# szhan227/text2protein

Measured on AMD Instinct MI355X. Metric: 6D backbone samples/sec (128-res, 1000-step), higher is better.
Workload: dtype f16; 1 GPU; cfg2: test_config.yml L=128 N=1000 chains/GPU=32 C=5 text_tokens=512 condition=none; step = 1 PC step (2 score evals + SDE updates); sample = 1000 PC steps; finite=True

## Files before the change

### text2protein_amd/csrc/attention.hip

```cpp
#include "t2p_kernels.h"

namespace t2p {

typedef float f32x16 __attribute__((ext_vector_type(16)));
typedef __bf16 bf16x8_t __attribute__((ext_vector_type(8)));
typedef _Float16 f16x8_t __attribute__((ext_vector_type(8)));

template <typename TC> struct AMma;
template <> struct AMma<bf16_t> {
  __device__ static inline void run(const uint4& a, const uint4& b, f32x16& c) {
    c = __builtin_amdgcn_mfma_f32_32x32x16_bf16(__builtin_bit_cast(bf16x8_t, a), __builtin_bit_cast(bf16x8_t, b), c, 0, 0, 0);
  }
};
template <> struct AMma<f16_t> {
  __device__ static inline void run(const uint4& a, const uint4& b, f32x16& c) {
    c = __builtin_amdgcn_mfma_f32_32x32x16_f16(__builtin_bit_cast(f16x8_t, a), __builtin_bit_cast(f16x8_t, b), c, 0, 0, 0);
  }
};

template <typename TC> __device__ inline uint32_t pack2(float a, float b);
template <> __device__ inline uint32_t pack2<bf16_t>(float a, float b) {
  return (uint32_t)f32_to_bf16_bits(a) | ((uint32_t)f32_to_bf16_bits(b) << 16);
}
template <> __device__ inline uint32_t pack2<f16_t>(float a, float b) {
// ... 181 lines not shown
  }

  const int qrow = q0 + lr;
  if (qrow < a.nq) {
    const float inv = 1.f / l;
    TC* orow = (TC*)a.out + (long)b * a.so_b + (long)qrow * a.ldo + (long)head * D;
#pragma unroll
    for (int tt = 0; tt < NT; ++tt)
#pragma unroll
      for (int g = 0; g < 4; ++g) {
        const int dv = tt * 32 + 8 * g + 4 * lh;
        uint2 u;
        u.x = pack2<TC>(o[tt][4 * g + 0] * inv, o[tt][4 * g + 1] * inv);
        u.y = pack2<TC>(o[tt][4 * g + 2] * inv, o[tt][4 * g + 3] * inv);
        *(uint2*)(orow + dv) = u;
      }
  }
}

template <typename TC, int D, bool VROW>
static int launch_flash_t(const FlashArgs& a, int B, int heads, hipStream_t s) {
  constexpr int smem = 2 * (64 * (D * 2 + 16) + (VROW ? 64 * (D == 32 ? 64 : (D == 64 ? 192 : 320)) : D * (64 * 2 + 8)));
  auto kern = attn_flash_kernel<TC, D, VROW>;
  T2P_TRY(ensure_dynamic_lds((const void*)kern, smem));
  dim3 grid((a.nq + 127) / 128, heads, B);
  hipEvent_t e0 = nullptr, e1 = nullptr;
  if (prof_on()) {
    T2P_HIP_CHECK(hipEventCreate(&e0));
    T2P_HIP_CHECK(hipEventCreate(&e1));
    T2P_HIP_CHECK(hipEventRecord(e0, s));
  }
  hipLaunchKernelGGL(kern, grid, dim3(256), smem, s, a);
  if (e0) {
    T2P_HIP_CHECK(hipEventRecord(e1, s));
    prof_attention(e0, e1, 4.0 * (double)a.nq * a.nk * D * heads * B);
  }
  T2P_HIP_CHECK(hipGetLastError());
  return T2P_OK;
}


struct StripArgs {
  const void* q; long ldq; long sq_b;
  const void* k; long ldk; long sk_b;
  const void* vt; long ldvt; long svt_b;
  void* out; long ldo; long so_b;
  int n;
  float scale_log2e;
  int ep, out_f32, r_lowp;
  const float* bias;
  const void* res; long ldr;
  float alpha;
  float* col_stats;
};

template <typename TC, int D, int NKT, bool FM = false>
__global__ __launch_bounds__(512) void attn_strip_kernel(const StripArgs a) {
  constexpr int QRS = D * 2 + 16;
  constexpr int KW = NKT * 32;
  constexpr int PRS = KW * 8 * 2 + 16;
  constexpr int CT = D / 256;
  constexpr int REGION = (64 * QRS > 64 * PRS) ? 64 * QRS : 64 * PRS;
  extern __shared__ __attribute__((aligned(16))) unsigned char smem[];
  float* st_max = (float*)(smem + REGION);
  float* st_sum = st_max + 8 * 64;

  const int tid = threadIdx.x, lane = tid & 63, wave = __builtin_amdgcn_readfirstlane(tid >> 6);
  const int lr = lane & 31, lh = lane >> 5;
  const int lid = xcd_logical_id((int)(blockIdx.x + gridDim.x * blockIdx.y), (int)(gridDim.x * gridDim.y));
  const int strip = lid % (int)gridDim.x, b = lid / (int)gridDim.x;
  const int q0 = strip * 64, n = a.n;
  const TC* Q = (const TC*)a.q + (long)b * a.sq_b;
  const TC* K = (const TC*)a.k + (long)b * a.sk_b;
  const TC* VT = (const TC*)a.vt + (long)b * a.svt_b;

  for (int i = tid; i < 64 * (D / 8); i += 512) {
    const int row = i / (D / 8), ch = i - row * (D / 8);
    uint4 v = make_uint4(0, 0, 0, 0);
    if (q0 + row < n) v = *(const uint4*)(Q + (long)(q0 + row) * a.ldq + ch * 8);
    *(uint4*)(smem + row * QRS + ch * 16) = v;
  }
  __syncthreads();

  const int key_w = wave * KW;
  const bool w_active = key_w < n;
  f32x16 sacc[NKT][2];
#pragma unroll
  for (int kt = 0; kt < NKT; ++kt)
#pragma unroll
    for (int qt = 0; qt < 2; ++qt)
#pragma unroll
      for (int v = 0; v < 16; ++v) sacc[kt][qt][v] = 0.f;
  if (w_active) {
    const TC* krow[NKT];
#pragma unroll
    for (int kt = 0; kt < NKT; ++kt) {
      int key = key_w + kt * 32 + lr;
      key = key < n ? key : n - 1;
      krow[kt] = K + (long)key * a.ldk + 16 * lh;
    }
#if defined(STRIP_FM_TIMING)
#define KLD(kt, S, j) (*(const uint4*)(K + ((((long)(key_w / 32 + (kt)) * (D / 32) + (S)) * 2 + (j)) * 64 + lane) * 8))
#else
#define KLD(kt, S, j) (FM ? *(const uint4*)(K + ((((long)(key_w / 32 + (kt)) * (D / 32) + (S)) * 2 + (j)) * 64 + lane) * 8) \
                          : *(const uint4*)(krow[kt] + 32 * (S) + 8 * (j)))
#endif
    const unsigned char* qb0 = smem + lr * QRS + 32 * lh;
    uint4 ka0[NKT][2], ka1[NKT][2];
#pragma unroll
    for (int kt = 0; kt < NKT; ++kt) {
      ka0[kt][0] = KLD(kt, 0, 0);
      ka0[kt][1] = KLD(kt, 0, 1);
    }
    auto sstep = [&](const uint4 (&ka)[NKT][2], int S) {
      uint4 qf[2][2];
#pragma unroll
      for (int qt = 0; qt < 2; ++qt)
#pragma unroll
        for (int j = 0; j < 2; ++j) qf[qt][j] = *(const uint4*)(qb0 + qt * 32 * QRS + S * 64 + j * 16);
#pragma unroll
      for (int kt = 0; kt < NKT; ++kt)
#pragma unroll
        for (int j = 0; j < 2; ++j)
#pragma unroll
          for (int qt = 0; qt < 2; ++qt) AMma<TC>::run(ka[kt][j], qf[qt][j], sacc[kt][qt]);
    };
    for (int S = 0; S < D / 32; S += 2) {
#pragma unroll
      for (int kt = 0; kt < NKT; ++kt) {
        ka1[kt][0] = KLD(kt, S + 1, 0);
        ka1[kt][1] = KLD(kt, S + 1, 1);
      }
      sstep(ka0, S);
      if (S + 2 < D / 32) {
#pragma unroll
        for (int kt = 0; kt < NKT; ++kt) {
          ka0[kt][0] = KLD(kt, S + 2, 0);
          ka0[kt][1] = KLD(kt, S + 2, 1);
        }
      }
      sstep(ka1, S + 1);
    }
  }

  float mloc[2] = {-INFINITY, -INFINITY};
  if (w_active) {
#pragma unroll
    for (int kt = 0; kt < NKT; ++kt) {
      const int kbase = key_w + kt * 32;
      if (kbase + 32 > n) {
#pragma unroll
        for (int v = 0; v < 16; ++v)
          if (kbase + (v & 3) + 8 * (v >> 2) + 4 * lh >= n) { sacc[kt][0][v] = -INFINITY; sacc[kt][1][v] = -INFINITY; }
      }
#pragma unroll
      for (int qt = 0; qt < 2; ++qt)
#pragma unroll
        for (int v = 0; v < 16; ++v) mloc[qt] = fmaxf(mloc[qt], sacc[kt][qt][v]);
    }
  }
#pragma unroll
  for (int qt = 0; qt < 2; ++qt) {
    mloc[qt] = fmaxf(mloc[qt], __shfl_xor(mloc[qt], 32, 64));
    if (lh == 0) st_max[wave * 64 + qt * 32 + lr] = mloc[qt];
  }
  __syncthreads();
  float mq[2], lsum[2] = {0.f, 0.f};
#pragma unroll
  for (int qt = 0; qt < 2; ++qt) {
    float m = st_max[qt * 32 + lr];
#pragma unroll
    for (int w = 1; w < 8; ++w) m = fmaxf(m, st_max[w * 64 + qt * 32 + lr]);
    mq[qt] = m * a.scale_log2e;
  }
  if (w_active) {
#pragma unroll
    for (int kt = 0; kt < NKT; ++kt)
#pragma unroll
      for (int qt = 0; qt < 2; ++qt) {
        unsigned char* prow = smem + (qt * 32 + lr) * PRS + (key_w + kt * 32 + 4 * lh) * 2;
#pragma unroll
        for (int g = 0; g < 4; ++g) {
          float e[4];
#pragma unroll
          for (int i = 0; i < 4; ++i) {
            e[i] = __builtin_amdgcn_exp2f(fmaf(sacc[kt][qt][4 * g + i], a.scale_log2e, -mq[qt]));
            lsum[qt] += e[i];
          }
          *(uint2*)(prow + 16 * g) = make_uint2(pack2<TC>(e[0], e[1]), pack2<TC>(e[2], e[3]));
        }
      }
  }
#pragma unroll
  for (int qt = 0; qt < 2; ++qt) {
    lsum[qt] += __shfl_xor(lsum[qt], 32, 64);
    if (lh == 0) st_sum[wave * 64 + qt * 32 + lr] = lsum[qt];
  }
  __syncthreads();
  float inv[2];
#pragma unroll
  for (int qt = 0; qt < 2; ++qt) {
    float l = st_sum[qt * 32 + lr];
#pragma unroll
    for (int w = 1; w < 8; ++w) l += st_sum[w * 64 + qt * 32 + lr];
    inv[qt] = 1.f / l;
  }

  f32x16 oacc[CT][2];
#pragma unroll
  for (int t = 0; t < CT; ++t)
#pragma unroll
    for (int qt = 0; qt < 2; ++qt)
#pragma unroll
      for (int v = 0; v < 16; ++v) oacc[t][qt][v] = 0.f;
  const int ch_w = wave * (D / 8);
  const TC* vrow[CT];
#pragma unroll
  for (int t = 0; t < CT; ++t) vrow[t] = VT + (long)(ch_w + t * 32 + lr) * a.ldvt + 16 * lh;
  const int nss = (n + 31) >> 5;
  auto vload = [&](int t, int S, int j) -> uint4 {
    const int key = 32 * S + 16 * lh + 8 * j;
#ifdef STRIP_FM_TIMING
    return key < n ? *(const uint4*)(VT + ((((long)(ch_w / 32 + t) * ((n + 31) >> 5) + S) * 2 + j) * 64 + lane) * 8) : make_uint4(0, 0, 0, 0);
#else
    if constexpr (FM) return *(const uint4*)(VT + ((((long)(ch_w / 32 + t) * (n >> 5) + S) * 2 + j) * 64 + lane) * 8);
    return key < n ? *(const uint4*)(vrow[t] + 32 * S + 8 * j) : make_uint4(0, 0, 0, 0);
#endif
  };
  uint4 va0[CT][2], va1[CT][2];
#pragma unroll
  for (int t = 0; t < CT; ++t) { va0[t][0] = vload(t, 0, 0); va0[t][1] = vload(t, 0, 1); }
  const unsigned char* pb0 = smem + lr * PRS + 32 * lh;
  auto pstep = [&](const uint4 (&va)[CT][2], int S) {
    uint4 pf[2][2];
#pragma unroll
    for (int qt = 0; qt < 2; ++qt)
#pragma unroll
      for (int j = 0; j < 2; ++j) pf[qt][j] = *(const uint4*)(pb0 + qt * 32 * PRS + S * 64 + j * 16);
#pragma unroll
    for (int t = 0; t < CT; ++t)
#pragma unroll
      for (int j = 0; j < 2; ++j)
#pragma unroll
        for (int qt = 0; qt < 2; ++qt) AMma<TC>::run(va[t][j], pf[qt][j], oacc[t][qt]);
  };
  for (int S = 0; S < nss; S += 2) {
    if (S + 1 < nss) {
#pragma unroll
      for (int t = 0; t < CT; ++t) { va1[t][0] = vload(t, S + 1, 0); va1[t][1] = vload(t, S + 1, 1); }
    }
    pstep(va0, S);
    if (S + 1 < nss) {
      if (S + 2 < nss) {
#pragma unroll
        for (int t = 0; t < CT; ++t) { va0[t][0] = vload(t, S + 2, 0); va0[t][1] = vload(t, S + 2, 1); }
      }
      pstep(va1, S + 1);
    }
  }

  if (!a.ep) {
#pragma unroll
    for (int qt = 0; qt < 2; ++qt) {
      const int qrow = q0 + qt * 32 + lr;
      if (qrow < n) {
        TC* orow = (TC*)a.out + (long)b * a.so_b + (long)qrow * a.ldo + ch_w;
#pragma unroll
        for (int t = 0; t < CT; ++t)
#pragma unroll
          for (int g = 0; g < 4; ++g) {
            uint2 u;
            u.x = pack2<TC>(oacc[t][qt][4 * g + 0] * inv[qt], oacc[t][qt][4 * g + 1] * inv[qt]);
            u.y = pack2<TC>(oacc[t][qt][4 * g + 2] * inv[qt], oacc[t][qt][4 * g + 3] * inv[qt]);
            *(uint2*)(orow + t * 32 + 8 * g + 4 * lh) = u;
          }
      }
    }
    return;
  }
#pragma unroll
  for (int t = 0; t < CT; ++t)
#pragma unroll
    for (int g = 0; g < 4; ++g) {
      const int ch = ch_w + t * 32 + 8 * g + 4 * lh;
      const float4 bs = a.bias ? *(const float4*)(a.bias + ch) : make_float4(0.f, 0.f, 0.f, 0.f);
      float cs[4] = {0.f, 0.f, 0.f, 0.f}, cq[4] = {0.f, 0.f, 0.f, 0.f};
#pragma unroll
      for (int qt = 0; qt < 2; ++qt) {
        const int qrow = q0 + qt * 32 + lr;
        if (qrow < n) {
          const long ro = (long)b * n * a.ldr + (long)qrow * a.ldr + ch;
          float r0 = 0.f, r1 = 0.f, r2 = 0.f, r3 = 0.f;
          if (a.res) {
            if (a.r_lowp) {
              union { uint2 u; TC e[4]; } x;
              x.u = *(const uint2*)((const TC*)a.res + ro);
              r0 = to_f32(x.e[0]); r1 = to_f32(x.e[1]); r2 = to_f32(x.e[2]); r3 = to_f32(x.e[3]);
            } else {
              const float4 x = *(const float4*)((const float*)a.res + ro);
              r0 = x.x; r1 = x.y; r2 = x.z; r3 = x.w;
            }
          }
          const float v0 = (oacc[t][qt][4 * g + 0] * inv[qt] + bs.x + r0) * a.alpha, v1 = (oacc[t][qt][4 * g + 1] * inv[qt] + bs.y + r1) * a.alpha;
          const float v2 = (oacc[t][qt][4 * g + 2] * inv[qt] + bs.z + r2) * a.alpha, v3 = (oacc[t][qt][4 * g + 3] * inv[qt] + bs.w + r3) * a.alpha;
          cs[0] += v0; cs[1] += v1; cs[2] += v2; cs[3] += v3;
          cq[0] += v0 * v0; cq[1] += v1 * v1; cq[2] += v2 * v2; cq[3] += v3 * v3;
          const long oo = (long)b * a.so_b + (long)qrow * a.ldo + ch;
          if (a.out_f32) *(float4*)((float*)a.out + oo) = make_float4(v0, v1, v2, v3);
          else *(uint2*)((TC*)a.out + oo) = make_uint2(pack2<TC>(v0, v1), pack2<TC>(v2, v3));
        }
      }
      if (a.col_stats) {
#pragma unroll
        for (int i = 0; i < 4; ++i)
#pragma unroll
          for (int sh = 1; sh < 32; sh <<= 1) { cs[i] += __shfl_xor(cs[i], sh, 64); cq[i] += __shfl_xor(cq[i], sh, 64); }
        if (lr == 0) {
          float* dst = a.col_stats + ((long)(b * (n >> 6) + strip) * D + ch) * 2;
          *(float4*)dst = make_float4(cs[0], cq[0], cs[1], cq[1]);
          *(float4*)(dst + 4) = make_float4(cs[2], cq[2], cs[3], cq[3]);
        }
      }
    }
}

bool g_attn_strip = true;
bool attention_strip_eligible(int dtype, int heads, int nq, int nk, int d, long ldq, long ldk, long ldvt, long ldo) {
  if (!g_attn_strip || dtype == DT_F32 || heads != 1 || nq != nk) return false;
  if (d != 256 && d != 512 && d != 1024) return false;
  if (nk < 8 || nk > 1024 || nk % 8 != 0) return false;
  if (d == 1024 && nk > 512) return false;
  return ldq % 8 == 0 && ldk % 8 == 0 && ldvt % 8 == 0 && ldvt >= nk && ldo % 4 == 0;
}

template <typename TC, int D, int NKT, bool FM = false>
static int launch_strip_t(const StripArgs& a, int B, hipStream_t s) {
  constexpr int QB = 64 * (D * 2 + 16), PB = 64 * (NKT * 32 * 8 * 2 + 16);
  constexpr int smem = (QB > PB ? QB : PB) + 2 * 8 * 64 * 4;
  static_assert(smem <= 160 * 1024, "attn_strip: LDS budget");
  auto kern = attn_strip_kernel<TC, D, NKT, FM>;
  T2P_TRY(ensure_dynamic_lds((const void*)kern, smem));
  hipEvent_t e0 = nullptr, e1 = nullptr;
  if (prof_on()) {
    T2P_HIP_CHECK(hipEventCreate(&e0));
    T2P_HIP_CHECK(hipEventCreate(&e1));
    T2P_HIP_CHECK(hipEventRecord(e0, s));
  }
  hipLaunchKernelGGL(kern, dim3((a.n + 63) / 64, B), dim3(512), smem, s, a);
  if (e0) {
    T2P_HIP_CHECK(hipEventRecord(e1, s));
    prof_attention(e0, e1, 4.0 * (double)a.n * a.n * D * B);
  }
  T2P_HIP_CHECK(hipGetLastError());
  return T2P_OK;
}

bool attention_strip_frag_major_ok(int dtype, int n, int d) {
  if ((dtype != DT_F16 && dtype != DT_BF16) || n % 32 != 0) return false;
  return (d == 512 && n > 512 && n <= 1024) || (d == 256 && n <= 256);
}
int launch_attention_strip(int dtype, const void* q, long ldq, const void* k, long ldk, const void* vt, long ldvt, void* out, long ldo,
                           int B, int n, int d, float scale, hipStream_t s, const StripEpilogue* ep) {
  T2P_REQUIRE(attention_strip_eligible(dtype, 1, n, n, d, ldq, ldk, ldvt, ldo), "wide-head attention: unsupported shape");
  T2P_REQUIRE(q && k && vt && out && B > 0 && scale > 0.f, "wide-head attention arguments");
  T2P_REQUIRE(((uintptr_t)q % 16) == 0 && ((uintptr_t)k % 16) == 0 && ((uintptr_t)vt % 16) == 0 && ((uintptr_t)out % 8) == 0,
              "wide-head attention: operands must be 16-byte aligned");
  StripArgs a;
  a.q = q; a.ldq = ldq; a.sq_b = (long)n * ldq;
  a.k = k; a.ldk = ldk; a.sk_b = (long)n * ldk;
  a.vt = vt; a.ldvt = ldvt; a.svt_b = (long)d * ldvt;
  a.out = out; a.ldo = ldo; a.so_b = (long)n * ldo;
  a.n = n;
  a.scale_log2e = scale * 1.44269504088896340736f;
  a.ep = ep ? 1 : 0; a.out_f32 = 0; a.r_lowp = 0; a.bias = nullptr; a.res = nullptr; a.ldr = 0; a.alpha = 1.f; a.col_stats = nullptr;
  if (ep) {
    T2P_REQUIRE(!ep->col_stats || n % 64 == 0, "wide-head attention: column statistics need whole 64-query strips");
    T2P_REQUIRE(!ep->residual || (ep->ldr % 4 == 0 && ((uintptr_t)ep->residual % 16) == 0), "wide-head attention: residual alignment");
    T2P_REQUIRE(((uintptr_t)out % 16) == 0 && ldo % 4 == 0, "wide-head attention: output alignment");
    a.out_f32 = ep->out_f32; a.r_lowp = ep->r_lowp; a.bias = ep->bias; a.res = ep->residual; a.ldr = ep->ldr; a.alpha = ep->alpha;
    a.col_stats = ep->col_stats;
  }
  const int nkt = n <= 256 ? 1 : (n <= 512 ? 2 : 4);
  if (ep && ep->frag_major) {
    T2P_REQUIRE(attention_strip_frag_major_ok(dtype, n, d), "wide-head attention: fragment-major operands need d = 512 with 512 < n <= 1024 or d = 256 with n <= 256, n % 32 == 0");
    a.sk_b = (long)n * d; a.svt_b = (long)n * d;
    if (d == 256) {
      if (dtype == DT_BF16) return launch_strip_t<bf16_t, 256, 1, true>(a, B, s);
      return launch_strip_t<f16_t, 256, 1, true>(a, B, s);
    }
    if (dtype == DT_BF16) return launch_strip_t<bf16_t, 512, 4, true>(a, B, s);
    return launch_strip_t<f16_t, 512, 4, true>(a, B, s);
  }
#define T2P_STRIP(TC, DD)                                                        \
  do {                                                                           \
    if (nkt == 1) return launch_strip_t<TC, DD, 1>(a, B, s);                     \
    if (nkt == 2) return launch_strip_t<TC, DD, 2>(a, B, s);                     \
    if constexpr (DD != 1024) return launch_strip_t<TC, DD, 4>(a, B, s);         \
  } while (0)
  if (dtype == DT_BF16) {
    if (d == 256) T2P_STRIP(bf16_t, 256);
    if (d == 512) T2P_STRIP(bf16_t, 512);
    if (d == 1024) T2P_STRIP(bf16_t, 1024);
  } else {
    if (d == 256) T2P_STRIP(f16_t, 256);
    if (d == 512) T2P_STRIP(f16_t, 512);
    if (d == 1024) T2P_STRIP(f16_t, 1024);
  }
#undef T2P_STRIP
  set_last_error("wide-head attention: no instantiation");
  return T2P_ERR_INVALID;
}

bool attention_flash_eligible(int dtype, int d, long ldq, long ldk, long ldvt, long ldo) {
  if (dtype == DT_F32) return false;
  if (d != 32 && d != 64 && d != 128) return false;
  return ldq % 8 == 0 && ldk % 8 == 0 && ldvt % 8 == 0 && ldo % 4 == 0;
}

int launch_attention_flash(int dtype, const void* q, long ldq, const void* k, long ldk, const void* vt, long ldvt,
                           void* out, int B, int heads, int nq, int nk, int d, float scale, hipStream_t s, bool v_rowmajor) {
  T2P_REQUIRE(attention_flash_eligible(dtype, d, ldq, ldk, ldvt, (long)heads * d), "flash attention: unsupported shape");
  T2P_REQUIRE(q && k && vt && out && B > 0 && heads > 0 && nq > 0 && nk > 0, "flash attention arguments");
  T2P_REQUIRE(scale > 0.f, "flash attention: the running maximum is taken on unscaled scores (scale must be positive)");
  T2P_REQUIRE(((uintptr_t)q % 16) == 0 && ((uintptr_t)k % 16) == 0 && ((uintptr_t)vt % 16) == 0 && ((uintptr_t)out % 8) == 0,
              "flash attention: operands must be 16-byte aligned");
  FlashArgs a;
  a.q = q; a.ldq = ldq; a.sq_b = (long)nq * ldq;
  a.k = k; a.ldk = ldk; a.sk_b = (long)nk * ldk;
  a.vt = vt; a.ldvt = ldvt; a.svt_b = v_rowmajor ? (long)nk * ldvt : (long)heads * d * ldvt;
  a.out = out; a.ldo = (long)heads * d; a.so_b = (long)nq * heads * d;
  a.nq = nq; a.nk = nk;
  a.scale_log2e = scale * 1.44269504088896340736f;
#define T2P_FLASH(TC, DD) return v_rowmajor ? launch_flash_t<TC, DD, true>(a, B, heads, s) : launch_flash_t<TC, DD, false>(a, B, heads, s)
  if (dtype == DT_BF16) {
    if (d == 32) T2P_FLASH(bf16_t, 32);
    if (d == 64) T2P_FLASH(bf16_t, 64);
    T2P_FLASH(bf16_t, 128);
  } else {
    if (d == 32) T2P_FLASH(f16_t, 32);
    if (d == 64) T2P_FLASH(f16_t, 64);
    T2P_FLASH(f16_t, 128);
  }
#undef T2P_FLASH
}

}
```

### text2protein_amd/csrc/capi.cpp

```cpp
#include <new>

#include "ddim.h"
#include "engine.h"
#include "sampler.h"
#include "train.h"

using namespace t2p;

#define API_BEGIN try {
#define API_END                                        \
  }                                                    \
  catch (const std::bad_alloc&) {                      \
    set_last_error("out of host memory");              \
    return T2P_ERR_STATE;                              \
  }                                                    \
  catch (const std::exception& ex) {                   \
    set_last_error(std::string("exception: ") + ex.what()); \
    return T2P_ERR_STATE;                              \
  }

namespace t2p { extern bool g_pre_conv_mfma, g_gn_apply_cols; void layer_profile_begin(); int layer_profile_end(std::string* out);
void debug_tap_set(int index, float* dst, long capacity); void debug_tap_shape(long out[4]); }
extern "C" {

// ... 640 lines not shown
  T2P_REQUIRE(npairs < (1u << 30), "encode_6d: too many block pairs");
  struct Scratch {
    int32_t* p = nullptr; hipStream_t s;
    ~Scratch() { if (p) { (void)hipStreamSynchronize(s); (void)hipFree(p); } }
  } dev;
  dev.s = s;
  T2P_HIP_CHECK(hipMalloc(&dev.p, up.size() * 4));
  T2P_HIP_CHECK(hipMemcpyAsync(dev.p, up.data(), up.size() * 4, hipMemcpyHostToDevice, s));
  return launch_encode6d(xyz, nres, atom_ok, batch, channels, L, dev.p, dev.p + 4 * (size_t)n_blocks, (int)npairs, coords_6d, mask_pair, s);
  API_END
}

int t2p_op_embedding_gather(const void* table, int table_dtype, const int32_t* ids, float* out, int64_t n_tokens, int dim, int vocab,
                            int32_t* bad_flag, void* stream) {
  API_BEGIN
  return launch_embedding_gather(table, table_dtype, ids, out, n_tokens, dim, vocab, bad_flag, (hipStream_t)stream);
  API_END
}

int t2p_op_apply_mask(float* x, const uint8_t* mask, const float* x_initial, int64_t n, void* stream) {
  API_BEGIN
  return launch_apply_mask(x, mask, x_initial, n, (hipStream_t)stream);
  API_END
}

int t2p_debug_set(int key, int value) {
  if (key == 10) { g_op_ws_bytes = (size_t)value << 20; return T2P_OK; }
  if (key == 11) { set_gemm_force_nsplit(value); return T2P_OK; }
  if (key == 12) { set_gemm_midsplit(value != 0); return T2P_OK; }
  if (key == 13) { g_gn_small = value != 0; return T2P_OK; }
  if (key == 14) { g_lowp_residual = value != 0; return T2P_OK; }
  if (key == 15) { set_gemm_thin_conv(value != 0); return T2P_OK; }
  if (key == 17) { g_gn_apply16 = value != 0; return T2P_OK; }
  if (key == 20) { g_layernorm16 = value != 0; return T2P_OK; }
  if (key == 21) { set_gemm_up4(value != 0); return T2P_OK; }
  if (key == 22) { set_gemm_deep_ring(value != 0); return T2P_OK; }
  if (key == 23) { set_gemm_fuse_shortcut(value != 0); return T2P_OK; }
  if (key == 25) { g_qkv_fused = value != 0; return T2P_OK; }
  if (key == 26) { t2p::g_pre_conv_mfma = value != 0; return T2P_OK; }
  if (key == 27) { t2p::g_gn_apply_cols = value != 0; return T2P_OK; }
  if (key == 28) { set_gemm_post_gn(value != 0); return T2P_OK; }
  if (key == 29) { t2p::g_attn_strip = value != 0; return T2P_OK; }
  if (key == 36) { t2p::g_small_conv = value != 0; return T2P_OK; }
  if (key == 38) { t2p::g_pre_conv_split = value != 0; return T2P_OK; }
  if (key == 39) { t2p::g_st_fuse = value != 0; return T2P_OK; }
  if (key == 40) { t2p::g_st_tail = value != 0; return T2P_OK; }
  if (key == 41) { t2p::g_small_conv_fm = value != 0; return T2P_OK; }
  if (key == 42) { t2p::g_st_ffpo = value != 0; return T2P_OK; }
  if (key == 43) { t2p::g_st_tail_rows = value; return T2P_OK; }
  if (key == 45) { t2p::g_attn_fm = value != 0; return T2P_OK; }
  if (key == 46) { t2p::g_attn_proj = value != 0; return T2P_OK; }
  if (key == 47) { set_gemm_dxs(value != 0); return T2P_OK; }
  if (key == 48) { t2p::g_train_plumbing16 = value != 0; return T2P_OK; }
  if (key == 34) { set_gemm_a_norm(value != 0); return T2P_OK; }
  if (key == 32) { g_attn_merged = value != 0; return T2P_OK; }
  if (key == 33) { g_ffpo_merged = value != 0; return T2P_OK; }
  if (key == 30) { set_gemm_split_consts(value, 0); return T2P_OK; }
  if (key == 31) { set_gemm_split_consts(0, value); return T2P_OK; }
  if (key == 0) set_gemm_dma(value != 0);
  else if (key == 1) {
#ifndef T2P_ABLATION
    if (value & ~(128 | 256 | 4096 | 8192)) {
      set_last_error("ablation bits that skip work exist only in a -DT2P_ABLATION build");
      return T2P_ERR_INVALID;
    }
#endif
    set_gemm_debug(value);
  }
  else if (key == 2) set_gemm_geom(value);
  else if (key == 3) set_gemm_splitk(value != 0);
  else if (key == 4) g_raw_copies = value != 0;
  else if (key == 5) g_flash_attention = value != 0;
  else if (key == 6) g_fuse_gn_stats = value != 0;
  else if (key == 7) g_fuse_geglu = value != 0;
  else if (key == 8) set_gemm_ring(value);
  else if (key == 9) g_lowp_h1 = value != 0;
  else return T2P_ERR_INVALID;
  return T2P_OK;
}

#ifdef T2P_ABLATION
extern "C" int t2p_ablation_dxs_stamps(unsigned long long* out, int n) { return t2p::dxs_stamps_read(out, n); }
#endif

int t2p_built_with_ablation(void) {
#ifdef T2P_ABLATION
  return 1;
#else
  return 0;
#endif
}

int t2p_profile_begin(void) {
  profile_begin();
  return T2P_OK;
}

int t2p_profile_end(double* out9) {
  API_BEGIN
  T2P_REQUIRE(out9, "null argument");
  double o[3][3];
  T2P_TRY(profile_end(o));
  for (int k = 0; k < 3; ++k)
    for (int j = 0; j < 3; ++j) out9[k * 3 + j] = o[k][j];
  return T2P_OK;
  API_END
// ... 56 lines not shown
```

### text2protein_amd/csrc/t2p_kernels.h

```cpp
#pragma once
#include "t2p_common.h"

namespace t2p {

struct GroupNormArgs {
  const float* x0 = nullptr; const float* x1 = nullptr;
  int C0 = 0, C1 = 0;
  int B = 0, HW = 0;
  int G = 0;
  float eps = 1e-6f;
  int lowp_dtype = DT_F32;
  float* partial = nullptr;
  float* stats = nullptr;
};
int gn_num_chunks(int HW);
int launch_gn_stats(const GroupNormArgs& a, hipStream_t s);

int launch_gn_finalize_cols(const float* cs0, const float* cs1, int C0, int C1, int B, int HW, int G, float eps,
                            float* stats, hipStream_t s);

struct GroupNormApplyArgs {
  const float* x0 = nullptr; const float* x1 = nullptr;
  int C0 = 0, C1 = 0, B = 0, H = 0, W = 0, G = 0;
  const float* stats = nullptr;
// ... 96 lines not shown
  int w_fm = 0;
  const void* X0 = nullptr; const void* X1 = nullptr;
  int CX0 = 0, CX1 = 0;
  const float* bias = nullptr;
  const float* bias_bn = nullptr;
  long ld_bn = 0;
  const void* R = nullptr;
  float alpha = 1.f;
  void* out = nullptr;
  int out_f32 = 0;
  float* col_stats = nullptr;
  void* normed = nullptr;
  const float* gn_gamma = nullptr; const float* gn_beta = nullptr;
  int groups = 0, gn_silu = 0;
  float gn_eps = 1e-6f;
};
extern bool g_small_conv;

struct StEntryArgs {
  int dtype = DT_F16;
  int B = 0, n = 0, C = 0;
  const void* x = nullptr;
  const float* cstats = nullptr;
  const float* gn_gamma = nullptr; const float* gn_beta = nullptr; int groups = 0; float gn_eps = 1e-6f;
  const void* w_in = nullptr; const float* b_in = nullptr;
  const float* ln_gamma = nullptr; const float* ln_beta = nullptr; float ln_eps = 1e-5f;
  const void* res = nullptr;
  const void* w_qkv = nullptr;
  int n2 = 0;
  const float* b2 = nullptr;
  int geglu = 0;
  const void* w3 = nullptr; const float* b3 = nullptr; const void* res3 = nullptr; void* y = nullptr; float* y_stats = nullptr;
  float* zero = nullptr; long zero_n = 0;
  void* t = nullptr;
  void* qkv = nullptr;
};
struct AttnProjArgs {
  int dtype = DT_F16;
  int B = 0, n = 0, C = 0;
  long npad = 0;
  const void* x = nullptr; const float* cstats = nullptr;
  const float* gn_gamma = nullptr; const float* gn_beta = nullptr; int groups = 0; float gn_eps = 1e-6f;
  const void* w_qk = nullptr; const float* b_qk = nullptr;
  const void* w_v = nullptr;
  void* qk = nullptr; void* vt = nullptr;
  void* k_fm = nullptr;
};
bool attn_proj_eligible(const AttnProjArgs& a);
int launch_attn_proj(const AttnProjArgs& a, hipStream_t s);
extern bool g_st_fuse;
extern bool g_small_conv_fm;
extern bool g_attn_proj;
extern bool g_attn_fm;
extern int g_st_tail_rows;
extern bool g_st_ffpo;
extern bool g_st_tail;
bool st_entry_eligible(const StEntryArgs& a);
int launch_st_entry(const StEntryArgs& a, hipStream_t s);
int launch_sf_frag_major(int dtype, const void* W, void* out, int N, int K, hipStream_t s);
bool small_conv_eligible(const SmallConvArgs& a);
int launch_small_conv_gn(const SmallConvArgs& a, hipStream_t s);

int launch_convert(const float* in, void* out, int dtype, long n, hipStream_t s);
int launch_widen(const void* in, int dtype, float* out, long n, hipStream_t s);
int launch_gather_label(const int* labels, const int* step_counter, const float* table, float* out, int B, int N,
                        hipStream_t s, const int* label_table = nullptr);
int launch_apply_mask(float* x, const unsigned char* mask, const float* x_initial, long n, hipStream_t s);
int launch_decode6d(const float* x, int B, int C, int L, float* clipped, float* absval, int* lengths, hipStream_t s);
int launch_encode6d(const float* xyz, const int* nres, const unsigned char* atom_ok, int B, int C, int L, const int* blocks, const int* pairs,
                    int npairs, float* coords_6d, unsigned char* mask_pair, hipStream_t s);
int launch_embedding_gather(const void* table, int dtype, const int* ids, float* out, long ntok, int dim, int vocab, int* bad, hipStream_t s);

}
```

Before: 0.6647 samples/s.

## Deepen attention strip load pipelining and stage epilogue through LDS

Adds a DEEP variant of the wide-head attention strip kernel. It keeps a deeper ring of K and V fragments in flight, pins the instruction schedule with sched_barrier, and issues the V prologue loads before the softmax so they overlap it. The epilogue can now stage the output and residual tiles through LDS and write them back as coalesced 16-byte rows, and the column-stat reductions use DPP/swizzle instead of shfl. Both paths are on by default behind new flags; the costs are more register pressure from the extra buffers and extra barriers in the epilogue.

Result: no change. 0.6693 samples/s (median of 6 runs) (+0.7%).

```diff
diff --git a/text2protein_amd/csrc/attention.hip b/text2protein_amd/csrc/attention.hip
--- a/text2protein_amd/csrc/attention.hip
+++ b/text2protein_amd/csrc/attention.hip
@@ -257,20 +257,91 @@
   const void* res; long ldr;
   float alpha;
   float* col_stats;
+  int stage_out, stage_res;
 };
 
-template <typename TC, int D, int NKT, bool FM = false>
+constexpr int strip_region_bytes(int D, int NKT) {
+  return 64 * ((D * 2 + 16) > (NKT * 32 * 8 * 2 + 16) ? (D * 2 + 16) : (NKT * 32 * 8 * 2 + 16));
+}
+constexpr bool strip_tile_fits(int D, int NKT, int es) { return 64 * (D * es + 16) <= strip_region_bytes(D, NKT); }
+
+template <int D, int ES, bool REGION_BUSY = true>
+__device__ __forceinline__ void strip_tile_fill(unsigned char* smem, const unsigned char* g, long ld_bytes, int rows, int tid) {
+  constexpr int TRS = D * ES + 16, CPR = D * ES / 16, NIT = 64 * CPR / 512;
+  uint4 r[NIT];
+#pragma unroll
+  for (int it = 0; it < NIT; ++it) {
+    const int i = tid + it * 512, row = i / CPR, c = i - row * CPR;
+    r[it] = make_uint4(0, 0, 0, 0);
+    if (row < rows) r[it] = *(const uint4*)(g + (long)row * ld_bytes + c * 16);
+  }
+  if constexpr (REGION_BUSY) __syncthreads();
+#pragma unroll
+  for (int it = 0; it < NIT; ++it) {
+    const int i = tid + it * 512, row = i / CPR, c = i - row * CPR;
+    *(uint4*)(smem + row * TRS + c * 16) = r[it];
+  }
+  __syncthreads();
+}
+
+template <int D, int ES>
+__device__ __forceinline__ void strip_tile_store(const unsigned char* smem, unsigned char* g, long ld_bytes, int rows, int tid) {
+  constexpr int TRS = D * ES + 16, CPR = D * ES / 16, NIT = 64 * CPR / 512;
+  __syncthreads();
+  uint4 r[NIT];
+#pragma unroll
+  for (int it = 0; it < NIT; ++it) {
+    const int i = tid + it * 512, row = i / CPR, c = i - row * CPR;
+    r[it] = *(const uint4*)(smem + row * TRS + c * 16);
+  }
+#pragma unroll
+  for (int it = 0; it < NIT; ++it) {
+    const int i = tid + it * 512, row = i / CPR, c = i - row * CPR;
+    if (row < rows) *(uint4*)(g + (long)row * ld_bytes + c * 16) = r[it];
+  }
+}
+
+#define STRIP_PIN() __builtin_amdgcn_sched_barrier(0x7cf)
+
+template <int SH> __device__ __forceinline__ float strip_lane_xor(float v) {
+  const int x = __builtin_bit_cast(int, v);
+  int r;
+  if constexpr (SH == 1) r = __builtin_amdgcn_update_dpp(0, x, 0xB1, 0xF, 0xF, false);
+  else if constexpr (SH == 2) r = __builtin_amdgcn_update_dpp(0, x, 0x4E, 0xF, 0xF, false);
+  else if constexpr (SH == 4) r = __builtin_amdgcn_update_dpp(0, x, 0x141, 0xF, 0xF, false);
+  else if constexpr (SH == 8) r = __builtin_amdgcn_update_dpp(0, x, 0x140, 0xF, 0xF, false);
+  else r = __builtin_amdgcn_ds_swizzle(x, 0x401F);
+  return __builtin_bit_cast(float, r);
+}
+
+#ifdef STRIP_TIMING
+__device__ unsigned long long g_strip_stamps[8];
+#define STRIP_STAMP(i) if (strip_t0) strip_st[i] = __builtin_amdgcn_s_memrealtime();
+#else
+#define STRIP_STAMP(i)
+#endif
+
+template <typename TC, int D, int NKT, bool FM = false, bool DEEP = false>
 __global__ __launch_bounds__(512) void attn_strip_kernel(const StripArgs a) {
   constexpr int QRS = D * 2 + 16;
   constexpr int KW = NKT * 32;
   constexpr int PRS = KW * 8 * 2 + 16;
   constexpr int CT = D / 256;
-  constexpr int REGION = (64 * QRS > 64 * PRS) ? 64 * QRS : 64 * PRS;
+  constexpr int REGION = strip_region_bytes(D, NKT);
+  constexpr int LA1 = !DEEP ? 2 : (NKT == 1 ? (D == 256 ? 4 : 8) : (NKT == 2 ? 4 : 2));
+  constexpr int LA2 = !DEEP ? 2 : 4;
+  static_assert(!DEEP || D != 1024, "attn_strip: no deep look-ahead at D = 1024");
+  static_assert((D / 32) % LA1 == 0, "attn_strip: pass 1 runs whole rounds of its buffers");
   extern __shared__ __attribute__((aligned(16))) unsigned char smem[];
   float* st_max = (float*)(smem + REGION);
   float* st_sum = st_max + 8 * 64;
 
   const int tid = threadIdx.x, lane = tid & 63, wave = __builtin_amdgcn_readfirstlane(tid >> 6);
+#ifdef STRIP_TIMING
+  const bool strip_t0 = blockIdx.x == 0 && blockIdx.y == 0 && tid == 0;
+  unsigned long long strip_st[8] = {0, 0, 0, 0, 0, 0, 0, 0};
+#endif
+  STRIP_STAMP(0)
   const int lr = lane & 31, lh = lane >> 5;
   const int lid = xcd_logical_id((int)(blockIdx.x + gridDim.x * blockIdx.y), (int)(gridDim.x * gridDim.y));
   const int strip = lid % (int)gridDim.x, b = lid / (int)gridDim.x;
@@ -279,13 +350,19 @@
   const TC* K = (const TC*)a.k + (long)b * a.sk_b;
   const TC* VT = (const TC*)a.vt + (long)b * a.svt_b;
 
-  for (int i = tid; i < 64 * (D / 8); i += 512) {
-    const int row = i / (D / 8), ch = i - row * (D / 8);
-    uint4 v = make_uint4(0, 0, 0, 0);
-    if (q0 + row < n) v = *(const uint4*)(Q + (long)(q0 + row) * a.ldq + ch * 8);
-    *(uint4*)(smem + row * QRS + ch * 16) = v;
-  }
-  __syncthreads();
+  if constexpr (DEEP) {
+    static_assert(QRS == D * 2 + 16, "attn_strip: query strip and 16-bit tile share a layout");
+    strip_tile_fill<D, 2, false>(smem, (const unsigned char*)(Q + (long)q0 * a.ldq), a.ldq * 2, n - q0, tid);
+  } else {
+    for (int i = tid; i < 64 * (D / 8); i += 512) {
+      const int row = i / (D / 8), ch = i - row * (D / 8);
+      uint4 v = make_uint4(0, 0, 0, 0);
+      if (q0 + row < n) v = *(const uint4*)(Q + (long)(q0 + row) * a.ldq + ch * 8);
+      *(uint4*)(smem + row * QRS + ch * 16) = v;
+    }
+    __syncthreads();
+  }
+  STRIP_STAMP(1)
 
   const int key_w = wave * KW;
   const bool w_active = key_w < n;
@@ -311,12 +388,14 @@
                           : *(const uint4*)(krow[kt] + 32 * (S) + 8 * (j)))
 #endif
     const unsigned char* qb0 = smem + lr * QRS + 32 * lh;
-    uint4 ka0[NKT][2], ka1[NKT][2];
-#pragma unroll
-    for (int kt = 0; kt < NKT; ++kt) {
-      ka0[kt][0] = KLD(kt, 0, 0);
-      ka0[kt][1] = KLD(kt, 0, 1);
-    }
+    uint4 ka[LA1][NKT][2];
+#pragma unroll
+    for (int i = 0; i < LA1 - 1; ++i)
+#pragma unroll
+      for (int kt = 0; kt < NKT; ++kt) {
+        ka[i][kt][0] = KLD(kt, i, 0);
+        ka[i][kt][1] = KLD(kt, i, 1);
+      }
     auto sstep = [&](const uint4 (&ka)[NKT][2], int S) {
       uint4 qf[2][2];
 #pragma unroll
@@ -330,94 +409,41 @@
 #pragma unroll
           for (int qt = 0; qt < 2; ++qt) AMma<TC>::run(ka[kt][j], qf[qt][j], sacc[kt][qt]);
     };
-    for (int S = 0; S < D / 32; S += 2) {
-#pragma unroll
-      for (int kt = 0; kt < NKT; ++kt) {
-        ka1[kt][0] = KLD(kt, S + 1, 0);
-        ka1[kt][1] = KLD(kt, S + 1, 1);
-      }
-      sstep(ka0, S);
-      if (S + 2 < D / 32) {
-#pragma unroll
-        for (int kt = 0; kt < NKT; ++kt) {
-          ka0[kt][0] = KLD(kt, S + 2, 0);
-          ka0[kt][1] = KLD(kt, S + 2, 1);
-        }
-      }
-      sstep(ka1, S + 1);
-    }
-  }
-
-  float mloc[2] = {-INFINITY, -INFINITY};
-  if (w_active) {
-#pragma unroll
-    for (int kt = 0; kt < NKT; ++kt) {
-      const int kbase = key_w + kt * 32;
-      if (kbase + 32 > n) {
-#pragma unroll
-        for (int v = 0; v < 16; ++v)
-          if (kbase + (v & 3) + 8 * (v >> 2) + 4 * lh >= n) { sacc[kt][0][v] = -INFINITY; sacc[kt][1][v] = -INFINITY; }
-      }
-#pragma unroll
-      for (int qt = 0; qt < 2; ++qt)
-#pragma unroll
-        for (int v = 0; v < 16; ++v) mloc[qt] = fmaxf(mloc[qt], sacc[kt][qt][v]);
-    }
-  }
-#pragma unroll
-  for (int qt = 0; qt < 2; ++qt) {
-    mloc[qt] = fmaxf(mloc[qt], __shfl_xor(mloc[qt], 32, 64));
-    if (lh == 0) st_max[wave * 64 + qt * 32 + lr] = mloc[qt];
-  }
-  __syncthreads();
-  float mq[2], lsum[2] = {0.f, 0.f};
-#pragma unroll
-  for (int qt = 0; qt < 2; ++qt) {
-    float m = st_max[qt * 32 + lr];
-#pragma unroll
-    for (int w = 1; w < 8; ++w) m = fmaxf(m, st_max[w * 64 + qt * 32 + lr]);
-    mq[qt] = m * a.scale_log2e;
-  }
-  if (w_active) {
-#pragma unroll
-    for (int kt = 0; kt < NKT; ++kt)
-#pragma unroll
-      for (int qt = 0; qt < 2; ++qt) {
-        unsigned char* prow = smem + (qt * 32 + lr) * PRS + (key_w + kt * 32 + 4 * lh) * 2;
-#pragma unroll
-        for (int g = 0; g < 4; ++g) {
-          float e[4];
-#pragma unroll
-          for (int i = 0; i < 4; ++i) {
-            e[i] = __builtin_amdgcn_exp2f(fmaf(sacc[kt][qt][4 * g + i], a.scale_log2e, -mq[qt]));
-            lsum[qt] += e[i];
+    if constexpr (!DEEP) {
+      for (int S0 = 0; S0 < D / 32; S0 += LA1) {
+#pragma unroll
+        for (int i = 0; i < LA1; ++i) {
+          const int S = S0 + i;
+          if (S + LA1 - 1 < D / 32) {
+#pragma unroll
+            for (int kt = 0; kt < NKT; ++kt) {
+              ka[(i + LA1 - 1) % LA1][kt][0] = KLD(kt, S + LA1 - 1, 0);
+              ka[(i + LA1 - 1) % LA1][kt][1] = KLD(kt, S + LA1 - 1, 1);
+            }
           }
-          *(uint2*)(prow + 16 * g) = make_uint2(pack2<TC>(e[0], e[1]), pack2<TC>(e[2], e[3]));
-        }
-      }
-  }
-#pragma unroll
-  for (int qt = 0; qt < 2; ++qt) {
-    lsum[qt] += __shfl_xor(lsum[qt], 32, 64);
-    if (lh == 0) st_sum[wave * 64 + qt * 32 + lr] = lsum[qt];
-  }
-  __syncthreads();
-  float inv[2];
-#pragma unroll
-  for (int qt = 0; qt < 2; ++qt) {
-    float l = st_sum[qt * 32 + lr];
-#pragma unroll
-    for (int w = 1; w < 8; ++w) l += st_sum[w * 64 + qt * 32 + lr];
-    inv[qt] = 1.f / l;
-  }
-
-  f32x16 oacc[CT][2];
-#pragma unroll
-  for (int t = 0; t < CT; ++t)
-#pragma unroll
-    for (int qt = 0; qt < 2; ++qt)
-#pragma unroll
-      for (int v = 0; v < 16; ++v) oacc[t][qt][v] = 0.f;
+          sstep(ka[i], S);
+        }
+      }
+    } else {
+      auto round = [&](int S0, bool last) {
+#pragma unroll
+        for (int i = 0; i < LA1; ++i) {
+          if (!last || i == 0) {
+#pragma unroll
+            for (int kt = 0; kt < NKT; ++kt) {
+              ka[(i + LA1 - 1) % LA1][kt][0] = KLD(kt, S0 + i + LA1 - 1, 0);
+              ka[(i + LA1 - 1) % LA1][kt][1] = KLD(kt, S0 + i + LA1 - 1, 1);
+            }
+            STRIP_PIN();
+          }
+          sstep(ka[i], S0 + i);
+        }
+      };
+      for (int S0 = 0; S0 + LA1 < D / 32; S0 += LA1) round(S0, false);
+      round(D / 32 - LA1, true);
+    }
+  }
+
   const int ch_w = wave * (D / 8);
   const TC* vrow[CT];
 #pragma unroll
@@ -432,9 +458,103 @@
     return key < n ? *(const uint4*)(vrow[t] + 32 * S + 8 * j) : make_uint4(0, 0, 0, 0);
 #endif
   };
-  uint4 va0[CT][2], va1[CT][2];
-#pragma unroll
-  for (int t = 0; t < CT; ++t) { va0[t][0] = vload(t, 0, 0); va0[t][1] = vload(t, 0, 1); }
+  auto vload_u = [&](int t, int S, int j) -> uint4 {
+    if constexpr (FM) {
+      const int Sc = S < nss ? S : nss - 1;
+      return *(const uint4*)(VT + ((((long)(ch_w / 32 + t) * (n >> 5) + Sc) * 2 + j) * 64 + lane) * 8);
+    }
+    const int key = 32 * S + 16 * lh + 8 * j;
+    const uint4 v = *(const uint4*)(vrow[t] + ((key < n ? key : n - 8) - 16 * lh));
+    return key < n ? v : make_uint4(0, 0, 0, 0);
+  };
+  uint4 va[LA2][CT][2];
+  auto vprologue = [&]() {
+#pragma unroll
+    for (int i = 0; i < LA2 - 1; ++i) {
+      if constexpr (DEEP) {
+#pragma unroll
+        for (int t = 0; t < CT; ++t) { va[i][t][0] = vload_u(t, i, 0); va[i][t][1] = vload_u(t, i, 1); }
+      } else if (i < nss) {
+#pragma unroll
+        for (int t = 0; t < CT; ++t) { va[i][t][0] = vload(t, i, 0); va[i][t][1] = vload(t, i, 1); }
+      }
+    }
+  };
+  if constexpr (DEEP) vprologue();
+
+  float mloc[2] = {-INFINITY, -INFINITY};
+  if (w_active) {
+#pragma unroll
+    for (int kt = 0; kt < NKT; ++kt) {
+      const int kbase = key_w + kt * 32;
+      if (kbase + 32 > n) {
+#pragma unroll
+        for (int v = 0; v < 16; ++v)
+          if (kbase + (v & 3) + 8 * (v >> 2) + 4 * lh >= n) { sacc[kt][0][v] = -INFINITY; sacc[kt][1][v] = -INFINITY; }
+      }
+#pragma unroll
+      for (int qt = 0; qt < 2; ++qt)
+#pragma unroll
+        for (int v = 0; v < 16; ++v) mloc[qt] = fmaxf(mloc[qt], sacc[kt][qt][v]);
+    }
+  }
+#pragma unroll
+  for (int qt = 0; qt < 2; ++qt) {
+    mloc[qt] = fmaxf(mloc[qt], __shfl_xor(mloc[qt], 32, 64));
+    if (lh == 0) st_max[wave * 64 + qt * 32 + lr] = mloc[qt];
+  }
+  __syncthreads();
+  STRIP_STAMP(2)
+  float mq[2], lsum[2] = {0.f, 0.f};
+#pragma unroll
+  for (int qt = 0; qt < 2; ++qt) {
+    float m = st_max[qt * 32 + lr];
+#pragma unroll
+    for (int w = 1; w < 8; ++w) m = fmaxf(m, st_max[w * 64 + qt * 32 + lr]);
+    mq[qt] = m * a.scale_log2e;
+  }
+  if (w_active) {
+#pragma unroll
+    for (int kt = 0; kt < NKT; ++kt)
+#pragma unroll
+      for (int qt = 0; qt < 2; ++qt) {
+        unsigned char* prow = smem + (qt * 32 + lr) * PRS + (key_w + kt * 32 + 4 * lh) * 2;
+#pragma unroll
+        for (int g = 0; g < 4; ++g) {
+          float e[4];
+#pragma unroll
+          for (int i = 0; i < 4; ++i) {
+            e[i] = __builtin_amdgcn_exp2f(fmaf(sacc[kt][qt][4 * g + i], a.scale_log2e, -mq[qt]));
+            lsum[qt] += e[i];
+          }
+          *(uint2*)(prow + 16 * g) = make_uint2(pack2<TC>(e[0], e[1]), pack2<TC>(e[2], e[3]));
+        }
+      }
+  }
+#pragma unroll
+  for (int qt = 0; qt < 2; ++qt) {
+    lsum[qt] += __shfl_xor(lsum[qt], 32, 64);
+    if (lh == 0) st_sum[wave * 64 + qt * 32 + lr] = lsum[qt];
+  }
+  __syncthreads();
+  STRIP_STAMP(3)
+  float inv[2];
+#pragma unroll
+  for (int qt = 0; qt < 2; ++qt) {
+    float l = st_sum[qt * 32 + lr];
+#pragma unroll
+    for (int w = 1; w < 8; ++w) l += st_sum[w * 64 + qt * 32 + lr];
+    inv[qt] = 1.f / l;
+  }
+
+  f32x16 oacc[CT][2];
+#pragma unroll
+  for (int t = 0; t < CT; ++t)
+#pragma unroll
+    for (int qt = 0; qt < 2; ++qt)
+#pragma unroll
+      for (int v = 0; v < 16; ++v) oacc[t][qt][v] = 0.f;
+  if constexpr (!DEEP) vprologue();
   const unsigned char* pb0 = smem + lr * PRS + 32 * lh;
   auto pstep = [&](const uint4 (&va)[CT][2], int S) {
     uint4 pf[2][2];
@@ -449,27 +569,56 @@
 #pragma unroll
         for (int qt = 0; qt < 2; ++qt) AMma<TC>::run(va[t][j], pf[qt][j], oacc[t][qt]);
   };
-  for (int S = 0; S < nss; S += 2) {
-    if (S + 1 < nss) {
-#pragma unroll
-      for (int t = 0; t < CT; ++t) { va1[t][0] = vload(t, S + 1, 0); va1[t][1] = vload(t, S + 1, 1); }
-    }
-    pstep(va0, S);
-    if (S + 1 < nss) {
-      if (S + 2 < nss) {
-#pragma unroll
-        for (int t = 0; t < CT; ++t) { va0[t][0] = vload(t, S + 2, 0); va0[t][1] = vload(t, S + 2, 1); }
-      }
-      pstep(va1, S + 1);
-    }
-  }
-
+  if constexpr (!DEEP) {
+    for (int S0 = 0; S0 < nss; S0 += LA2) {
+#pragma unroll
+      for (int i = 0; i < LA2; ++i) {
+        const int S = S0 + i;
+        if (S < nss) {
+          if (S + LA2 - 1 < nss) {
+#pragma unroll
+            for (int t = 0; t < CT; ++t) {
+              va[(i + LA2 - 1) % LA2][t][0] = vload(t, S + LA2 - 1, 0);
+              va[(i + LA2 - 1) % LA2][t][1] = vload(t, S + LA2 - 1, 1);
+            }
+          }
+          pstep(va[i], S);
+        }
+      }
+    }
+  } else {
+    int S0 = 0;
+    for (; S0 + LA2 <= nss; S0 += LA2) {
+#pragma unroll
+      for (int i = 0; i < LA2; ++i) {
+#pragma unroll
+        for (int t = 0; t < CT; ++t) {
+          va[(i + LA2 - 1) % LA2][t][0] = vload_u(t, S0 + i + LA2 - 1, 0);
+          va[(i + LA2 - 1) % LA2][t][1] = vload_u(t, S0 + i + LA2 - 1, 1);
+        }
+        STRIP_PIN();
+        pstep(va[i], S0 + i);
+      }
+    }
+#pragma unroll
+    for (int i = 0; i < LA2 - 1; ++i)
+      if (S0 + i < nss) pstep(va[i], S0 + i);
+  }
+
+  const int rows = n - q0 < 64 ? n - q0 : 64;
+  unsigned char* const out_strip = (unsigned char*)a.out + ((long)b * a.so_b + (long)q0 * a.ldo) * (a.ep && a.out_f32 ? 4 : 2);
+#ifdef STRIP_TIMING
+  __syncthreads();
+  STRIP_STAMP(4)
+#endif
   if (!a.ep) {
+    if (a.stage_out) __syncthreads();
 #pragma unroll
     for (int qt = 0; qt < 2; ++qt) {
       const int qrow = q0 + qt * 32 + lr;
       if (qrow < n) {
         TC* orow = (TC*)a.out + (long)b * a.so_b + (long)qrow * a.ldo + ch_w;
+        unsigned char* trow = smem + (qt * 32 + lr) * (D * 2 + 16) + ch_w * 2;
 #pragma unroll
         for (int t = 0; t < CT; ++t)
 #pragma unroll
@@ -477,32 +626,68 @@
             uint2 u;
             u.x = pack2<TC>(oacc[t][qt][4 * g + 0] * inv[qt], oacc[t][qt][4 * g + 1] * inv[qt]);
             u.y = pack2<TC>(oacc[t][qt][4 * g + 2] * inv[qt], oacc[t][qt][4 * g + 3] * inv[qt]);
-            *(uint2*)(orow + t * 32 + 8 * g + 4 * lh) = u;
+            if (a.stage_out) *(uint2*)(trow + (t * 32 + 8 * g + 4 * lh) * 2) = u;
+            else *(uint2*)(orow + t * 32 + 8 * g + 4 * lh) = u;
           }
       }
     }
+    if (a.stage_out) strip_tile_store<D, 2>(smem, out_strip, a.ldo * 2, rows, tid);
+#ifdef STRIP_TIMING
+    __builtin_amdgcn_s_waitcnt(0);
+    __syncthreads();
+    STRIP_STAMP(5)
+    if (strip_t0) {
+#pragma unroll
+      for (int i = 0; i < 8; ++i) g_strip_stamps[i] = strip_st[i];
+    }
+#endif
     return;
   }
+  const int tes = a.out_f32 ? 4 : 2, trs = D * tes + 16;
+  constexpr bool BIAS_AHEAD = CT < 4;
+  float4 bsv[BIAS_AHEAD ? CT : 1][4];
+  if (a.stage_out) {
+    if constexpr (BIAS_AHEAD) {
+#pragma unroll
+      for (int t = 0; t < CT; ++t)
+#pragma unroll
+        for (int g = 0; g < 4; ++g)
+          bsv[t][g] = a.bias ? *(const float4*)(a.bias + ch_w + t * 32 + 8 * g + 4 * lh) : make_float4(0.f, 0.f, 0.f, 0.f);
+    }
+    if (a.stage_res) {
+      const unsigned char* res_strip = (const unsigned char*)a.res + ((long)b * n + q0) * a.ldr * tes;
+      if (a.out_f32) {
+        if constexpr (strip_tile_fits(D, NKT, 4)) strip_tile_fill<D, 4>(smem, res_strip, a.ldr * 4, rows, tid);
+      } else {
+        strip_tile_fill<D, 2>(smem, res_strip, a.ldr * 2, rows, tid);
+      }
+    } else {
+      __syncthreads();
+    }
+  }
+  STRIP_STAMP(6)
 #pragma unroll
   for (int t = 0; t < CT; ++t)
 #pragma unroll
     for (int g = 0; g < 4; ++g) {
       const int ch = ch_w + t * 32 + 8 * g + 4 * lh;
-      const float4 bs = a.bias ? *(const float4*)(a.bias + ch) : make_float4(0.f, 0.f, 0.f, 0.f);
+      const float4 bs = BIAS_AHEAD && a.stage_out ? bsv[BIAS_AHEAD ? t : 0][g]
+                                                  : (a.bias ? *(const float4*)(a.bias + ch) : make_float4(0.f, 0.f, 0.f, 0.f));
       float cs[4] = {0.f, 0.f, 0.f, 0.f}, cq[4] = {0.f, 0.f, 0.f, 0.f};
 #pragma unroll
       for (int qt = 0; qt < 2; ++qt) {
         const int qrow = q0 + qt * 32 + lr;
         if (qrow < n) {
           const long ro = (long)b * n * a.ldr + (long)qrow * a.ldr + ch;
+          unsigned char* tp = smem + (qt * 32 + lr) * trs + ch * tes;
           float r0 = 0.f, r1 = 0.f, r2 = 0.f, r3 = 0.f;
           if (a.res) {
             if (a.r_lowp) {
               union { uint2 u; TC e[4]; } x;
-              x.u = *(const uint2*)((const TC*)a.res + ro);
+              x.u = a.stage_res ? *(const uint2*)tp : *(const uint2*)((const TC*)a.res + ro);
               r0 = to_f32(x.e[0]); r1 = to_f32(x.e[1]); r2 = to_f32(x.e[2]); r3 = to_f32(x.e[3]);
             } else {
-              const float4 x = *(const float4*)((const float*)a.res + ro);
+              const float4 x = a.stage_res ? *(const float4*)tp : *(const float4*)((const float*)a.res + ro);
               r0 = x.x; r1 = x.y; r2 = x.z; r3 = x.w;
             }
           }
@@ -511,15 +696,33 @@
           cs[0] += v0; cs[1] += v1; cs[2] += v2; cs[3] += v3;
           cq[0] += v0 * v0; cq[1] += v1 * v1; cq[2] += v2 * v2; cq[3] += v3 * v3;
           const long oo = (long)b * a.so_b + (long)qrow * a.ldo + ch;
-          if (a.out_f32) *(float4*)((float*)a.out + oo) = make_float4(v0, v1, v2, v3);
-          else *(uint2*)((TC*)a.out + oo) = make_uint2(pack2<TC>(v0, v1), pack2<TC>(v2, v3));
+          if (a.out_f32) {
+            const float4 o = make_float4(v0, v1, v2, v3);
+            if (a.stage_out) *(float4*)tp = o;
+            else *(float4*)((float*)a.out + oo) = o;
+          } else {
+            const uint2 o = make_uint2(pack2<TC>(v0, v1), pack2<TC>(v2, v3));
+            if (a.stage_out) *(uint2*)tp = o;
+            else *(uint2*)((TC*)a.out + oo) = o;
+          }
         }
       }
       if (a.col_stats) {
-#pragma unroll
-        for (int i = 0; i < 4; ++i)
-#pragma unroll
-          for (int sh = 1; sh < 32; sh <<= 1) { cs[i] += __shfl_xor(cs[i], sh, 64); cq[i] += __shfl_xor(cq[i], sh, 64); }
+        if (a.stage_out) {
+#pragma unroll
+          for (int i = 0; i < 4; ++i) {
+            cs[i] += strip_lane_xor<1>(cs[i]); cq[i] += strip_lane_xor<1>(cq[i]);
+            cs[i] += strip_lane_xor<2>(cs[i]); cq[i] += strip_lane_xor<2>(cq[i]);
+            cs[i] += strip_lane_xor<4>(cs[i]); cq[i] += strip_lane_xor<4>(cq[i]);
+            cs[i] += strip_lane_xor<8>(cs[i]); cq[i] += strip_lane_xor<8>(cq[i]);
+            cs[i] += strip_lane_xor<16>(cs[i]); cq[i] += strip_lane_xor<16>(cq[i]);
+          }
+        } else {
+#pragma unroll
+          for (int i = 0; i < 4; ++i)
+#pragma unroll
+            for (int sh = 1; sh < 32; sh <<= 1) { cs[i] += __shfl_xor(cs[i], sh, 64); cq[i] += __shfl_xor(cq[i], sh, 64); }
+        }
         if (lr == 0) {
           float* dst = a.col_stats + ((long)(b * (n >> 6) + strip) * D + ch) * 2;
           *(float4*)dst = make_float4(cs[0], cq[0], cs[1], cq[1]);
@@ -527,6 +730,23 @@
         }
       }
     }
+  STRIP_STAMP(7)
+  if (a.stage_out) {
+    if (a.out_f32) {
+      if constexpr (strip_tile_fits(D, NKT, 4)) strip_tile_store<D, 4>(smem, out_strip, a.ldo * 4, rows, tid);
+    } else {
+      strip_tile_store<D, 2>(smem, out_strip, a.ldo * 2, rows, tid);
+    }
+  }
+#ifdef STRIP_TIMING
+  __builtin_amdgcn_s_waitcnt(0);
+  __syncthreads();
+  STRIP_STAMP(5)
+  if (strip_t0) {
+#pragma unroll
+    for (int i = 0; i < 8; ++i) g_strip_stamps[i] = strip_st[i];
+  }
+#endif
 }
 
 bool g_attn_strip = true;
@@ -538,12 +758,14 @@
   return ldq % 8 == 0 && ldk % 8 == 0 && ldvt % 8 == 0 && ldvt >= nk && ldo % 4 == 0;
 }
 
-template <typename TC, int D, int NKT, bool FM = false>
-static int launch_strip_t(const StripArgs& a, int B, hipStream_t s) {
-  constexpr int QB = 64 * (D * 2 + 16), PB = 64 * (NKT * 32 * 8 * 2 + 16);
-  constexpr int smem = (QB > PB ? QB : PB) + 2 * 8 * 64 * 4;
+bool g_attn_strip_tail = true;
+bool g_attn_strip_deep = true;
+
+template <typename TC, int D, int NKT, bool FM, bool DEEP>
+static int launch_strip_k(const StripArgs& a, int B, hipStream_t s) {
+  constexpr int smem = strip_region_bytes(D, NKT) + 2 * 8 * 64 * 4;
   static_assert(smem <= 160 * 1024, "attn_strip: LDS budget");
-  auto kern = attn_strip_kernel<TC, D, NKT, FM>;
+  auto kern = attn_strip_kernel<TC, D, NKT, FM, DEEP>;
   T2P_TRY(ensure_dynamic_lds((const void*)kern, smem));
   hipEvent_t e0 = nullptr, e1 = nullptr;
   if (prof_on()) {
@@ -558,6 +780,18 @@
   }
   T2P_HIP_CHECK(hipGetLastError());
   return T2P_OK;
+}
+
+template <typename TC, int D, int NKT, bool FM = false>
+static int launch_strip_t(const StripArgs& a0, int B, hipStream_t s) {
+  StripArgs a = a0;
+  const int es = a.ep && a.out_f32 ? 4 : 2;
+  a.stage_out = g_attn_strip_tail && (es == 2 || strip_tile_fits(D, NKT, 4)) && (a.ldo * es) % 16 == 0 && ((uintptr_t)a.out % 16) == 0;
+  a.stage_res = a.stage_out && a.res && (a.r_lowp ? 2 : 4) == es && (a.ldr * es) % 16 == 0 && ((uintptr_t)a.res % 16) == 0;
+  if constexpr (D != 1024) {
+    if (g_attn_strip_deep) return launch_strip_k<TC, D, NKT, FM, true>(a, B, s);
+  }
+  return launch_strip_k<TC, D, NKT, FM, false>(a, B, s);
 }
 
 bool attention_strip_frag_major_ok(int dtype, int n, int d) {
@@ -578,6 +812,7 @@
   a.n = n;
   a.scale_log2e = scale * 1.44269504088896340736f;
   a.ep = ep ? 1 : 0; a.out_f32 = 0; a.r_lowp = 0; a.bias = nullptr; a.res = nullptr; a.ldr = 0; a.alpha = 1.f; a.col_stats = nullptr;
+  a.stage_out = 0; a.stage_res = 0;
   if (ep) {
     T2P_REQUIRE(!ep->col_stats || n % 64 == 0, "wide-head attention: column statistics need whole 64-query strips");
     T2P_REQUIRE(!ep->residual || (ep->ldr % 4 == 0 && ((uintptr_t)ep->residual % 16) == 0), "wide-head attention: residual alignment");
@@ -650,3 +885,10 @@
 }
 
 }
+
+#ifdef STRIP_TIMING
+extern "C" int t2p_strip_stamps(unsigned long long* out8) {
+  if (hipDeviceSynchronize() != hipSuccess) return 1;
+  return hipMemcpyFromSymbol(out8, HIP_SYMBOL(t2p::g_strip_stamps), 8 * sizeof(unsigned long long)) == hipSuccess ? 0 : 1;
+}
+#endif
diff --git a/text2protein_amd/csrc/capi.cpp b/text2protein_amd/csrc/capi.cpp
--- a/text2protein_amd/csrc/capi.cpp
+++ b/text2protein_amd/csrc/capi.cpp
@@ -716,6 +716,8 @@
   if (key == 46) { t2p::g_attn_proj = value != 0; return T2P_OK; }
   if (key == 47) { set_gemm_dxs(value != 0); return T2P_OK; }
   if (key == 48) { t2p::g_train_plumbing16 = value != 0; return T2P_OK; }
+  if (key == 49) { t2p::g_attn_strip_tail = value != 0; return T2P_OK; }
+  if (key == 50) { t2p::g_attn_strip_deep = value != 0; return T2P_OK; }
   if (key == 34) { set_gemm_a_norm(value != 0); return T2P_OK; }
   if (key == 32) { g_attn_merged = value != 0; return T2P_OK; }
   if (key == 33) { g_ffpo_merged = value != 0; return T2P_OK; }
diff --git a/text2protein_amd/csrc/t2p_kernels.h b/text2protein_amd/csrc/t2p_kernels.h
--- a/text2protein_amd/csrc/t2p_kernels.h
+++ b/text2protein_amd/csrc/t2p_kernels.h
@@ -172,6 +172,8 @@
 extern bool g_small_conv_fm;
 extern bool g_attn_proj;
 extern bool g_attn_fm;
+extern bool g_attn_strip_tail;
+extern bool g_attn_strip_deep;
 extern int g_st_tail_rows;
 extern bool g_st_ffpo;
 extern bool g_st_tail;
```
